# NikolasMarkou/blind_image_denoising

Hardware: AMD Instinct MI355X
Metric: denoised images/sec (256x256x3) + MAE vs ref, resnet_1x18 (higher is better)
Workload: dtype f16x2 split (hi+lo, fp32 accumulate)

## Files before the change

blind_image_denoising_amd/csrc/fused_h3w.hip:

```cpp
#include "h3v_core.h"
#include "h3_bands.h"
#include "base_rows.h"

#ifndef H3W_PRIO_SET
#define H3W_PRIO_SET 0
#endif
#if H3W_PRIO_SET == 1
#define H3W_PRIO_A1 0
#define H3W_PRIO_B1 1
#define H3W_PRIO_A2 2
#define H3W_PRIO_B2 3
#elif H3W_PRIO_SET == 2
#define H3W_PRIO_A1 3
#define H3W_PRIO_B1 2
#define H3W_PRIO_A2 1
#define H3W_PRIO_B2 0
#elif H3W_PRIO_SET == 3
#define H3W_PRIO_A1 0
#define H3W_PRIO_B1 2
#define H3W_PRIO_A2 0
#define H3W_PRIO_B2 2
#elif H3W_PRIO_SET == 4
#define H3W_PRIO_A1 2
#define H3W_PRIO_B1 0
#define H3W_PRIO_A2 2
#define H3W_PRIO_B2 0
#endif
#ifndef H3W_PRIO_A1
#define H3W_PRIO_A1 1
#endif
#ifndef H3W_PRIO_B1
#define H3W_PRIO_B1 1
#endif
#ifndef H3W_PRIO_A2
#define H3W_PRIO_A2 1
#endif
#ifndef H3W_PRIO_B2
#define H3W_PRIO_B2 1
#endif

#ifndef H3W_XCD_ORDER
#define H3W_XCD_ORDER 1
#endif

struct H3WGeom {
    static constexpr int NG = 9, GW = 16 * NG;
    static constexpr int G = 3;
    static constexpr int NR = 3, NW = 12, NT = 768;
    static constexpr int SW = 128;
    static constexpr int PITCH = (GW + 2) * 16;
    static constexpr int NRX0 = 5, NRM = 2, NRX1 = 3, NRO = 2;
    static constexpr int PD = 3;
    static constexpr int UNROLL = 6;
    static constexpr int X0_PLANE = (NRX0 * PITCH + 255) / 256 * 256, M_PLANE = (NRM * PITCH + 255) / 256 * 256;
    static constexpr int X1_PLANE = (NRX1 * PITCH + 255) / 256 * 256;
    static constexpr int OUT_PLANE = GW * 16, OUT_SLOT = 4 * OUT_PLANE;
    static constexpr int X0_OFF = 0, M1_OFF = X0_OFF + 4 * X0_PLANE, X1_OFF = M1_OFF + 4 * M_PLANE, M2_OFF = X1_OFF + 4 * X1_PLANE;
    static constexpr int OUT_OFF = M2_OFF + 4 * M_PLANE, LDS_BYTES = OUT_OFF + NRO * OUT_SLOT;
    static constexpr int BIN_RING = 4, BIN_ROWPX = GW + 4;
    static constexpr int BIN_SLOT = 2 * BIN_ROWPX * 8;
    static constexpr int BIN_OFF = LDS_BYTES, BWA_OFF = BIN_OFF + BIN_RING * BIN_SLOT, BINVS_OFF = BWA_OFF + 3 * 64 * 16;
    static constexpr int BRED_OFF = BINVS_OFF + 16, LDS_BYTES_BASE = BRED_OFF + NT * 4;
    static_assert(LDS_BYTES_BASE <= 160 * 1024 && BIN_OFF % 16 == 0 && BIN_SLOT % 16 == 0 && LDS_BYTES_BASE % 16 == 0, "LDS (producer)");
    static constexpr int LEAD = 12;
    static constexpr int NSTAMP = 4;
    static_assert(UNROLL % NRM == 0 && UNROLL % NRO == 0 && UNROLL % NRX1 == 0 && UNROLL % 3 == 0, "static slots");
    static_assert(NRX0 == PD + 2, "x0 ring: rows s-1 (residual), s (conv1a), s+1 (landed), s+2, s+3 (in flight)");
    static_assert(LDS_BYTES <= 160 * 1024, "LDS");
    static_assert(3 * X0_PLANE + NRX0 * PITCH < 65536, "fragment offsets fit the 16-bit ds offset");
};

struct H3WTile : BandUnit {
    int X0, X1;
    int G0;
    int D0, D1;
};

__device__ __forceinline__ H3WTile h3w_tile(const FusedH3WArgs& a, const int t)
{
    H3WTile r{bf_band_unit<H3W_XCD_ORDER != 0>(a, t)};
    r.X0 = r.sx * H3WGeom::SW;
    r.X1 = min(a.W, r.X0 + H3WGeom::SW);
    r.G0 = min(max(r.X0 - 8, 0), max(a.W - H3WGeom::GW, 0));
    r.D0 = max(0, (r.X0 - 4) & ~7);
    r.D1 = min(a.W, (r.X1 + 4 + 7) & ~7);
    return r;
}

template <int INP>
struct H3WRoleA {
    using Gm = H3WGeom;
    const char* tin;
    char* tmid;
    h8 w[13];
    f32x4 acc[Gm::G][3];
    int rp, rs;
    int wr;
    float inv_s, relu_floor;
    float lane_scale[Gm::G];
    bool skip_last = false;

    __device__ __forceinline__ void init(const void* wimg, const FusedH3WArgs& a, const float* aux, const int lane, const int gc0)
    {
        const int q = lane >> 4;
#pragma unroll
        for (int i = 0; i < 13; ++i) w[i] = reinterpret_cast<const h8*>(wimg)[bf_band_wimage(a, i) * 64 + lane];
        inv_s = aux[0];
        relu_floor = a.act1_relu ? 0.f : -__builtin_inff();
        rp = (q & 1) * INP + (gc0 + (q >> 1)) * 16;
        rs = ((q & 1) + 2 * (q >> 1)) * INP + (gc0 + 2) * 16;
        wr = (q >> 1) * Gm::M_PLANE + (gc0 + 1) * 16 + (q & 1) * 8;
#pragma unroll
        for (int g = 0; g < Gm::G; ++g)
#pragma unroll
            for (int k = 0; k < 3; ++k) acc[g][k] = (f32x4){0.f, 0.f, 0.f, 0.f};
    }
    __device__ __forceinline__ void set_tile(const H3WTile& t, const int W, const int gc0)
    {
#pragma unroll
        for (int g = 0; g < Gm::G; ++g) lane_scale[g] = (t.G0 + gc0 + 16 * g < W) ? inv_s : 0.f;
    }

    __device__ __forceinline__ H3VFrag load(const int islot_bytes, const int g) const
    {
        H3VFrag f;
        const char* p = tin + rp + islot_bytes;
        f.ph = *reinterpret_cast<const h8*>(p + g * 256);
        f.pl = *reinterpret_cast<const h8*>(p + g * 256 + 2 * INP);
        f.s = *reinterpret_cast<const h8*>(tin + rs + islot_bytes + g * 256);
        return f;
    }

    __device__ __forceinline__ H3VEpi<true> epilogue(const int g, const int mslot, const f32x4 v, const bool rowok) const
    {
        H3VEpi<true> e;
        e.v = v;
        e.sc = rowok ? lane_scale[g] : 0.f;
        e.floor_ = relu_floor;
        e.p = tmid + wr + mslot * Gm::PITCH + g * 256;
        e.lo_off = 2 * Gm::M_PLANE;
        return e;
    }

    template <int J, class Epi>
    __device__ __forceinline__ void mfmas(const int g, const int a1, const int a2, const H3VFrag& cur, f32x4& c0, Epi* epi)
    {
        if constexpr (J < 15) {
            constexpr int k = J / 3, which = J % 3;
            if (!(H3V_ABLATE & 8) && !(skip_last && g == Gm::G - 1)) {
                if constexpr (which == 0) acc[g][a2] = h3v_mfma(cur, w, 2, k, acc[g][a2]);
                else if constexpr (which == 1) acc[g][a1] = h3v_mfma(cur, w, 1, k, acc[g][a1]);
                else c0 = h3v_mfma(cur, w, 0, k, c0);
            } else if (J == 0) {
                acc[g][a2][0] += (float)cur.ph[0] + (float)cur.pl[1] + (float)cur.s[2];
            }
            __builtin_amdgcn_sched_barrier(0);
            if constexpr (J >= 2) {
                if (epi) epi->template pair<J - 2>();
            }
            mfmas<J + 1>(g, a1, a2, cur, c0, epi);
        }
    }

    template <int PH, class Hook>
    __device__ __forceinline__ void step(const int islot_bytes, const bool rowok, Hook& hook)
    {
        constexpr int a0 = PH % 3, a1 = (PH + 2) % 3, a2 = (PH + 1) % 3;
        constexpr int mslot = PH % Gm::NRM;
        H3VFrag cur = load(islot_bytes, 0);
#pragma unroll
        for (int g = 0; g < Gm::G; ++g) {
            H3VFrag nx;
            if (g + 1 < Gm::G) nx = load(islot_bytes, g + 1);
            __builtin_amdgcn_sched_barrier(0);
            f32x4 c0 = {0.f, 0.f, 0.f, 0.f};
            if (g > 0) {
                H3VEpi<true> e = epilogue(g - 1, mslot, acc[g - 1][a2], rowok);
                mfmas<0>(g, a1, a2, cur, c0, &e);
            } else {
                mfmas<0>(g, a1, a2, cur, c0, (H3VEpi<true>*)nullptr);
                hook.after_first_group();
                __builtin_amdgcn_sched_barrier(0);
            }
            acc[g][a0] = c0;
            if (g + 1 < Gm::G) cur = nx;
        }
        H3VEpi<true> e = epilogue(Gm::G - 1, mslot, bf_acc_ready(acc[Gm::G - 1][a2]), rowok);
        e.all();
    }
};

template <int RESP, int OUTP>
struct H3WRoleB {
    using Gm = H3WGeom;
    const char* tmid;
    const char* tres;
    char* tout;
    h8 w[13];
    f32x4 acc[Gm::G][3];
    int rp, rs;
    int rr;
    int wo;
    float inv_s2;
    f32x4 shs;
    float lane_scale[Gm::G];
    bool skip_last = false;

    __device__ __forceinline__ void init(const void* wimg, const FusedH3WArgs& a, const float* aux, const int lane, const int gc0,
                                         const bool out_is_ring)
    {
        const int q = lane >> 4;
#pragma unroll
        for (int i = 0; i < 13; ++i) w[i] = reinterpret_cast<const h8*>(wimg)[bf_band_wimage(a, i) * 64 + lane];
        inv_s2 = aux[48];
        shs = *reinterpret_cast<const f32x4*>(aux + 32 + q * 4) * (1.0f / inv_s2);
        rp = (q & 1) * Gm::M_PLANE + (gc0 + (q >> 1)) * 16;
        rs = ((q & 1) + 2 * (q >> 1)) * Gm::M_PLANE + (gc0 + 2) * 16;
        rr = ((q & 1) + 2 * (q >> 1)) * RESP + (gc0 + 1) * 16;
        wo = (q >> 1) * OUTP + (gc0 + (out_is_ring ? 1 : 0)) * 16 + (q & 1) * 8;
#pragma unroll
        for (int g = 0; g < Gm::G; ++g)
#pragma unroll
            for (int k = 0; k < 3; ++k) acc[g][k] = (f32x4){0.f, 0.f, 0.f, 0.f};
    }
    __device__ __forceinline__ void set_tile(const H3WTile& t, const int W, const int gc0)
    {
#pragma unroll
        for (int g = 0; g < Gm::G; ++g) lane_scale[g] = (t.G0 + gc0 + 16 * g < W) ? inv_s2 : 0.f;
    }

    __device__ __forceinline__ H3VFrag load(const int mslot, const int g) const
    {
        H3VFrag f;
        const int o = mslot * Gm::PITCH + g * 256;
        f.ph = *reinterpret_cast<const h8*>(tmid + rp + o);
        f.pl = *reinterpret_cast<const h8*>(tmid + rp + o + 2 * Gm::M_PLANE);
        f.s = *reinterpret_cast<const h8*>(tmid + rs + o);
        return f;
    }
    __device__ __forceinline__ h8 load_res(const int xslot_bytes, const int g) const
    {
        return *reinterpret_cast<const h8*>(tres + rr + xslot_bytes + g * 256);
    }

    __device__ __forceinline__ H3VEpi<false> epilogue(const int g, const int oslot_bytes, const f32x4 accv, const bool rowok) const
    {
        H3VEpi<false> e;
        e.v = accv;
        e.sc = rowok ? lane_scale[g] : 0.f;
        e.floor_ = 0.f;
        e.p = tout + wo + oslot_bytes + g * 256;
        e.lo_off = 2 * OUTP;
        return e;
    }

    template <int J, class Epi>
    __device__ __forceinline__ void mfmas(const int g, const int a1, const int a2, const H3VFrag& cur, const h8 xr, f32x4& c0, Epi* epi)
    {
        if constexpr (J < 16) {
            if (!(H3V_ABLATE & 4) && !(skip_last && g == Gm::G - 1)) {
                if constexpr (J == 0) {
                    c0 = MFMA_H(w[12], xr, shs);
                } else {
                    constexpr int k = (J - 1) / 3, which = (J - 1) % 3;
                    if constexpr (which == 0) acc[g][a2] = h3v_mfma(cur, w, 2, k, acc[g][a2]);
                    else if constexpr (which == 1) acc[g][a1] = h3v_mfma(cur, w, 1, k, acc[g][a1]);
                    else c0 = h3v_mfma(cur, w, 0, k, c0);
                }
            } else if (J == 0) {
                acc[g][a2][0] += (float)cur.ph[0] + (float)cur.pl[1] + (float)cur.s[2] + (float)xr[3];
            }
            __builtin_amdgcn_sched_barrier(0);
            if constexpr (J >= 2) {
                if (epi) epi->template pair<J - 2>();
            }
            mfmas<J + 1>(g, a1, a2, cur, xr, c0, epi);
        }
    }

    template <int PH, class Hook>
    __device__ __forceinline__ void step(const int xslot_bytes, const int oslot_bytes, const bool rowok, Hook& hook)
    {
        constexpr int mslot = (PH + 1) % Gm::NRM;
        constexpr int a0 = PH % 3, a1 = (PH + 2) % 3, a2 = (PH + 1) % 3;
        H3VFrag cur = load(mslot, 0);
        h8 xr = load_res(xslot_bytes, 0);
#pragma unroll
        for (int g = 0; g < Gm::G; ++g) {
            H3VFrag nx;
            h8 xn;
            if (g + 1 < Gm::G) {
                nx = load(mslot, g + 1);
                xn = load_res(xslot_bytes, g + 1);
            }
            __builtin_amdgcn_sched_barrier(0);
            f32x4 c0;
            if (g > 0) {
                H3VEpi<false> e = epilogue(g - 1, oslot_bytes, acc[g - 1][a2], rowok);
                mfmas<0>(g, a1, a2, cur, xr, c0, &e);
            } else {
                mfmas<0>(g, a1, a2, cur, xr, c0, (H3VEpi<false>*)nullptr);
                hook.after_first_group();
                __builtin_amdgcn_sched_barrier(0);
            }
            acc[g][a0] = c0;
            if (g + 1 < Gm::G) {
                cur = nx;
                xr = xn;
            }
        }
        H3VEpi<false> e = epilogue(Gm::G - 1, oslot_bytes, bf_acc_ready(acc[Gm::G - 1][a2]), rowok);
        e.all();
    }
};

#ifndef H3W_MEM_ROLES
#define H3W_MEM_ROLES 0
#endif
constexpr int h3w_mem_kind(const int role)
{
    constexpr int loader[4] = {2, 0, 1, 3}, storer[4] = {0, 1, 0, 0};
    return role == loader[H3W_MEM_ROLES] ? 1 : (role == storer[H3W_MEM_ROLES] ? 2 : 0);
}

template <int KIND>
struct H3WMem {
    __device__ __forceinline__ H3WMem(const FusedH3WArgs&, char*, const char*, int, unsigned) {}
    __device__ __forceinline__ void set_tile(const H3WTile&, int) {}
    __device__ __forceinline__ void prologue(const H3WTile&) {}
    __device__ __forceinline__ void begin(const H3WTile&, int, int) {}
    __device__ __forceinline__ void after_first_group() {}
    __device__ __forceinline__ void end() {}
    __device__ __forceinline__ void finish() {}
};

template <>
struct H3WMem<1> {
    using Gm = H3WGeom;
    const FusedH3WArgs& a;
    char* tin;
    int piece;
    unsigned plane_g;
    unsigned col_off;
    bool active;
    int dslot;

    __device__ __forceinline__ H3WMem(const FusedH3WArgs& a_, char* tx0, const char*, const int rw, const unsigned pg)
        : a(a_), tin(tx0), piece(rw), plane_g(pg), col_off(0), active(false), dslot(0) {}
    __device__ __forceinline__ void set_tile(const H3WTile& t, const int lane)
    {
        const int c = t.G0 + 64 * piece + lane;
        active = (c >= t.D0) & (c < t.D1) & (64 * piece + lane < Gm::GW);
        col_off = (unsigned)c * 16u;
    }
    __device__ __forceinline__ void dma_row(const H3WTile& t, const int r, const int slot) const
    {
        if (H3V_ABLATE & 1) return;
        const int y = t.y(r - 4);
        const bool ok = (y >= 0) & (y < a.H) & (r < t.nrows + 8);
#pragma unroll
        for (int plane = 0; plane < 4; ++plane) {
            const char* src = ok ? reinterpret_cast<const char*>(a.in) + t.img + (size_t)plane * plane_g + (size_t)y * a.W * 16 + col_off
                                 : reinterpret_cast<const char*>(a.zeros);
            char* dst = tin + plane * Gm::X0_PLANE + slot * Gm::PITCH + (1 + 64 * piece) * 16;
            if (active) h3_dma16(src, dst);
        }
    }
    static constexpr int INFLIGHT = 2 * 4;
    __device__ __forceinline__ void wait_landed() const { __builtin_amdgcn_s_waitcnt(h3_vmcnt((H3V_ABLATE & 1) ? 0 : INFLIGHT)); }
    __device__ __forceinline__ void prologue(const H3WTile& t)
    {
#pragma unroll
        for (int r = 0; r < Gm::PD; ++r) dma_row(t, r, r);
        wait_landed();
        dslot = Gm::PD;
    }
    __device__ __forceinline__ void begin(const H3WTile& t, const int s, int)
    {
        dma_row(t, s + Gm::PD, dslot);
        dslot = h3v_wrap(dslot + 1, Gm::NRX0);
    }
    __device__ __forceinline__ void after_first_group() {}
    __device__ __forceinline__ void end() { wait_landed(); }
    __device__ __forceinline__ void finish() { __builtin_amdgcn_s_waitcnt(h3_vmcnt(0)); }
};

template <>
struct H3WMem<2> {
    using Gm = H3WGeom;
    const FusedH3WArgs& a;
    const char* tout;
    int first, np;
    unsigned plane_g;
    int st_off[3];
    unsigned g_off[3];
    bool okc[3];
    h8 rec[3];
    bool have;
    char* image;
    size_t row_off;

    __device__ __forceinline__ H3WMem(const FusedH3WArgs& a_, char*, const char* tout_, const int rw, const unsigned pg)
        : a(a_), tout(tout_), first(3 * rw), np(rw < 2 ? 3 : 2), plane_g(pg), have(false), image(nullptr), row_off(0) {}
    __device__ __forceinline__ void set_tile(const H3WTile& t, const int lane)
    {
#pragma unroll
        for (int i = 0; i < 3; ++i) {
            const int p = first + i, plane = p >> 1, c = t.X0 + 64 * (p & 1) + lane;
            okc[i] = (i < np) & (c < t.X1);
            st_off[i] = plane * Gm::OUT_PLANE + (c - t.G0) * 16;
            g_off[i] = (unsigned)plane * plane_g + (unsigned)c * 16u;
        }
    }
    __device__ __forceinline__ void prologue(const H3WTile&) {}
    __device__ __forceinline__ void begin(const H3WTile& t, const int s, const int PH)
    {
        const int k = s - Gm::LEAD, oslot = (PH + 1) % Gm::NRO;
        have = (k >= 0) & (k < t.nrows) & !(H3V_ABLATE & 2);
        if (!have) return;
        image = reinterpret_cast<char*>(a.out) + t.img;
        row_off = (size_t)t.y(k) * a.W * 16;
#pragma unroll
        for (int i = 0; i < 3; ++i)
            if (i < np) rec[i] = *reinterpret_cast<const h8*>(tout + oslot * Gm::OUT_SLOT + st_off[i]);
    }
    __device__ __forceinline__ void after_first_group()
    {
        if (!have) return;
#pragma unroll
        for (int i = 0; i < 3; ++i)
            if (okc[i]) h3_stream_store16(image, 4u * plane_g, row_off, g_off[i], rec[i]);
    }
    __device__ __forceinline__ void end() {}
    __device__ __forceinline__ void finish() {}
};

template <>
struct H3WMem<3> {
    using Gm = H3WGeom;
    const FusedH3WArgs& a;
    const char* tout;
    int half;
    int st_off;
    int col;
    bool okc;

    __device__ __forceinline__ H3WMem(const FusedH3WArgs& a_, char*, const char* tout_, const int rw, const unsigned)
        : a(a_), tout(tout_), half(rw), st_off(0), col(0), okc(false) {}
    __device__ __forceinline__ void set_tile(const H3WTile& t, const int lane)
    {
        col = t.X0 + 64 * half + lane;
        okc = (half < 2) & (col < t.X1) & (col < a.Wo);
        st_off = (col - t.G0) * 16;
    }
    __device__ __forceinline__ void prologue(const H3WTile&) {}
    __device__ __forceinline__ void begin(const H3WTile& t, const int s, const int PH)
    {
        const int k = s - Gm::LEAD, oslot = (PH + 1) % Gm::NRO;
        bool have = (half < 2) & (k >= 0) & (k < t.nrows) & !(H3V_ABLATE & 2);
        if (have) have = t.y(k) < a.Ho;
        if (!have) return;
        char* orow = reinterpret_cast<char*>(a.head_out) + ((size_t)t.b * a.Ho + (size_t)t.y(k)) * a.Wo * 3 * (a.head_u8 ? 1 : 4);
        const char* src = tout + oslot * Gm::OUT_SLOT + st_off;
        float h0 = 0.f, h1 = 0.f, h2 = 0.f;
#pragma unroll
        for (int hf = 0; hf < 2; ++hf) {
            const h8 hi = *reinterpret_cast<const h8*>(src + hf * Gm::OUT_PLANE), lo = *reinterpret_cast<const h8*>(src + (2 + hf) * Gm::OUT_PLANE);
#pragma unroll
            for (int c = 0; c < 8; ++c) {
                const float v = (float)hi[c] + (float)lo[c];
                const f32x4 w = *reinterpret_cast<const f32x4*>(a.head_wh + (hf * 8 + c) * 4);
                h0 = fmaf(v, w.x, h0);
                h1 = fmaf(v, w.y, h1);
                h2 = fmaf(v, w.z, h2);
            }
        }
        const bool finite = fabsf(h0) <= 3.0e38f && fabsf(h1) <= 3.0e38f && fabsf(h2) <= 3.0e38f;
        if (!finite && a.status) atomicOr(a.status, BF_STATUS_F16_RANGE);
        float r[3] = {h0, h1, h2};
#pragma unroll
        for (int o = 0; o < 3; ++o) {
            float v = (1.0f - 2.0f / (__expf(4.0f * r[o]) + 1.0f)) * 0.51f;
            if (a.denormalize) v = (fminf(fmaxf(v, -0.5f), 0.5f) + 0.5f) * (a.v_max - a.v_min) + a.v_min;
            r[o] = v;
        }
        if (!okc) return;
        if (a.head_u8) {
            unsigned char* p = reinterpret_cast<unsigned char*>(orow) + (size_t)col * 3;
#pragma unroll
            for (int o = 0; o < 3; ++o) p[o] = (unsigned char)fminf(fmaxf(rintf(r[o]), 0.f), 255.f);
        } else {
            float* p = reinterpret_cast<float*>(orow) + (size_t)col * 3;
#pragma unroll
            for (int o = 0; o < 3; ++o) p[o] = r[o];
        }
        __builtin_amdgcn_sched_barrier(0);
    }
    __device__ __forceinline__ void after_first_group() {}
    __device__ __forceinline__ void end() {}
    __device__ __forceinline__ void finish() {}
};

#ifndef H3W_BASE_SPREAD
#define H3W_BASE_SPREAD 1
#endif
constexpr int h3w_base_groups(const int role)
{
    return H3W_BASE_SPREAD == 0 ? (role == 2 ? 3 : 0) : (H3W_BASE_SPREAD == 1 ? (role >= 1 ? 1 : 0) : (role <= 2 ? 1 : 0));
}
constexpr int h3w_base_first_group(const int role, const int rw)
{
    return H3W_BASE_SPREAD == 0 ? 3 * rw : (H3W_BASE_SPREAD == 1 ? 3 * (role - 1) + rw : 3 * role + rw);
}
constexpr bool h3w_base_fetches(const int role) { return role == 2; }

template <int NGW, bool FETCH>
struct H3WProducer {
    using Gm = H3WGeom;
    const FusedH3WArgs& a;
    char* tx0;
    char* tring;
    const char* twa;
    int g0, fw;
    float inv_s, floor_;
    int wr;
    int fo;
    int col0;
    int px, xcol;
    const uint8_t* img;
    unsigned raw[3];
    BrPixel rawp;
    int dslot;

    __device__ __forceinline__ H3WProducer(const FusedH3WArgs& a_, char* lds, const int g0_, const int fw_)
        : a(a_), tx0(lds + Gm::X0_OFF), tring(lds + Gm::BIN_OFF), twa(lds + Gm::BWA_OFF), g0(g0_), fw(fw_), wr(0), fo(0), col0(0),
          px(0), xcol(0), img(nullptr), raw{0u, 0u, 0u}, rawp{false, false}, dslot(0)
    {
        inv_s = *reinterpret_cast<const float*>(lds + Gm::BINVS_OFF);
        floor_ = a.base_relu ? 0.f : -__builtin_inff();
    }
    __device__ __forceinline__ void set_tile(const H3WTile& t, const int lane)
    {
        const int n = lane & 15, q = lane >> 4, gc0 = 16 * g0 + n;
        wr = (q >> 1) * Gm::X0_PLANE + (gc0 + 1) * 16 + (q & 1) * 8;
        const int p = gc0 + 2 * (q & 1);
        fo = ((p & 1) * Gm::BIN_ROWPX + (p & ~1)) * 8;
        twa = tx0 - Gm::X0_OFF + Gm::BWA_OFF + lane * 16;
        col0 = t.G0 + gc0;
        px = 64 * fw + lane;
        xcol = t.G0 - 1 + px;
        img = reinterpret_cast<const uint8_t*>(a.base_u8) + (size_t)t.b * a.Hs * a.Ws * 3;
    }
    __device__ __forceinline__ void request(const H3WTile& t, const int u)
    {
        const int yy = t.ybase + u - 5;
        const bool need = (px < Gm::GW + 2) & (u <= t.nrows + 9);
        rawp = br_pixel(yy, xcol, a.H, a.W, a.Hs, a.Ws);
        rawp.inside &= need;
        rawp.colour &= need;
        if (rawp.colour) {
            const uint8_t* p = img + ((size_t)yy * a.Ws + xcol) * 3;
            raw[0] = p[0];
            raw[1] = p[1];
            raw[2] = p[2];
        }
    }
    __device__ __forceinline__ void commit(const int u)
    {
        if (px >= Gm::GW + 2) return;
        const h4 v = br_record(rawp, raw[0], raw[1], raw[2]);
        h4* row = reinterpret_cast<h4*>(tring + (u & (Gm::BIN_RING - 1)) * Gm::BIN_SLOT);
        row[px] = v;
        if (px > 0) row[Gm::BIN_ROWPX + px - 1] = v;
    }
    __device__ __forceinline__ void produce(const H3WTile& t, const int r, const int slot)
    {
        if (r >= t.nrows + 8) return;
        const int y = t.y(r - 4);
        const bool rowok = (y >= 0) & (y < a.H);
        f32x4 acc[NGW];
#pragma unroll
        for (int g = 0; g < NGW; ++g) acc[g] = (f32x4){0.f, 0.f, 0.f, 0.f};
#pragma unroll
        for (int dy = 0; dy < 3; ++dy) {
            const h8 wa = *reinterpret_cast<const h8*>(twa + dy * 64 * 16);
            const char* row = tring + ((r + dy) & (Gm::BIN_RING - 1)) * Gm::BIN_SLOT + fo;
#pragma unroll
            for (int g = 0; g < NGW; ++g) acc[g] = MFMA_H(wa, *reinterpret_cast<const h8*>(row + g * 128), acc[g]);
        }
#pragma unroll
        for (int g = 0; g < NGW; ++g) {
            H3VEpi<true> e;
            e.v = bf_acc_ready(acc[g]);
            e.sc = (rowok & (col0 + 16 * g < a.W)) ? inv_s : 0.f;
            e.floor_ = floor_;
            e.p = tx0 + wr + slot * Gm::PITCH + g * 256;
            e.lo_off = 2 * Gm::X0_PLANE;
            e.all();
        }
    }
    __device__ __forceinline__ void fill(const H3WTile& t)
    {
        if constexpr (FETCH) {
#pragma unroll
            for (int u = 0; u < Gm::BIN_RING; ++u) {
                request(t, u);
                commit(u);
            }
            request(t, Gm::BIN_RING);
        }
    }
    __device__ __forceinline__ void prologue(const H3WTile& t)
    {
        produce(t, 0, 0);
        dslot = 1;
    }
    __device__ __forceinline__ void begin(const H3WTile& t, const int s)
    {
        if constexpr (FETCH) {
            commit(s + 4);
            request(t, s + 5);
        }
        produce(t, s + 1, dslot);
        dslot = h3v_wrap(dslot + 1, Gm::NRX0);
        __builtin_amdgcn_sched_barrier(0);
    }
};

template <>
struct H3WProducer<0, false> {
    __device__ __forceinline__ H3WProducer(const FusedH3WArgs&, char*, int, int) {}
    __device__ __forceinline__ void set_tile(const H3WTile&, int) {}
    __device__ __forceinline__ void fill(const H3WTile&) {}
    __device__ __forceinline__ void prologue(const H3WTile&) {}
    __device__ __forceinline__ void begin(const H3WTile&, int) {}
};

template <bool HEAD, bool BASE>
constexpr int h3w_hook_kind(const int role)
{
    const int k = h3w_mem_kind(role);
    return (HEAD && k == 2) ? 3 : ((BASE && k == 1) ? 0 : k);
}

template <bool HEAD, bool BASE>
__global__ __launch_bounds__(H3WGeom::NT, 3) void fused_block2_h3w_kernel(FusedH3WArgs a)
{
    using Gm = H3WGeom;
    extern __shared__ __attribute__((aligned(16))) char h3w_lds[];
    char* tx0 = h3w_lds + Gm::X0_OFF;
    char* tm1 = h3w_lds + Gm::M1_OFF;
    char* tx1 = h3w_lds + Gm::X1_OFF;
    char* tm2 = h3w_lds + Gm::M2_OFF;
    char* tout = h3w_lds + Gm::OUT_OFF;
    const int tid = threadIdx.x, lane = tid & 63;
    const int wave = __builtin_amdgcn_readfirstlane(tid >> 6);
    const int n = lane & 15;
    const int role = wave / Gm::NR, rw = wave - role * Gm::NR;
    const unsigned plane_g = (unsigned)a.H * (unsigned)a.W * 16u;
    const int gc0 = 16 * Gm::G * rw + n;

    if (BASE && a.status && blockIdx.x == 0 && tid == 0) *a.status = 0;
    for (int i = tid * 16; i < (BASE ? Gm::LDS_BYTES_BASE : Gm::LDS_BYTES); i += Gm::NT * 16)
        *reinterpret_cast<f32x4*>(h3w_lds + i) = (f32x4){0.f, 0.f, 0.f, 0.f};
    __syncthreads();
    if constexpr (BASE) {
        const float bs = br_weight_scale(a.base_w, reinterpret_cast<float*>(h3w_lds + Gm::BRED_OFF));
        if (wave == 0) {
#pragma unroll
            for (int dy = 0; dy < 3; ++dy)
                *reinterpret_cast<h8*>(h3w_lds + Gm::BWA_OFF + (dy * 64 + lane) * 16) = br_operand(a.base_w, bs, dy, lane);
            if (lane == 0) *reinterpret_cast<float*>(h3w_lds + Gm::BINVS_OFF) = 1.0f / bs;
        }
        __syncthreads();
    }

#if H3V_ABLATE & 32
    unsigned long long stamp_sum[Gm::NSTAMP] = {0, 0, 0, 0}, stamp_prev, real0;
    asm volatile("s_memrealtime %0\n\ts_memtime %1\n\ts_waitcnt lgkmcnt(0)" : "=s"(real0), "=s"(stamp_prev)::"memory");
#endif

#define H3W_ROW_IN_IMAGE(k) ((t.y(k) >= 0) & (t.y(k) < a.H))
#define H3W_BAND(R, M, P, ACTIVE, STEP)                                                                         \
    for (int ti = blockIdx.x; ti < a.ntiles; ti += gridDim.x) {                                               \
        const H3WTile t = h3w_tile(a, ti);                                                                    \
        R.set_tile(t, a.W, gc0);                                                                              \
        M.set_tile(t, lane);                                                                                  \
        P.set_tile(t, lane);                                                                                  \
        if constexpr (BASE) {                                      \
            P.fill(t);                                                                                        \
            h3v_barrier();                                                                                    \
        }                                                                                                     \
        P.prologue(t);                                                                                        \
        M.prologue(t);                                                                                        \
        h3v_barrier();                                                 \
        const int nsteps = t.nrows + Gm::LEAD;                                                                \
        int slot5 = 0;                                                                           \
        for (int s0 = 0; s0 < nsteps; s0 += Gm::UNROLL) {                                                     \
            H3W_ONE(0, M, P, ACTIVE, STEP); H3W_ONE(1, M, P, ACTIVE, STEP); H3W_ONE(2, M, P, ACTIVE, STEP);   \
            H3W_ONE(3, M, P, ACTIVE, STEP); H3W_ONE(4, M, P, ACTIVE, STEP); H3W_ONE(5, M, P, ACTIVE, STEP);   \
        }                                                                                                     \
        M.finish();                                                                                           \
        h3v_barrier();                                                                                        \
    }
#define H3W_ONE(PH, M, P, ACTIVE, STEP)                                                                         \
    do {                                                                                                      \
        const int s = s0 + PH;                                                                                \
        P.begin(t, s);                                                                                        \
        M.begin(t, s, PH);                                                                                    \
        if (ACTIVE(s)) { STEP(PH); }                                                                          \
        else M.after_first_group();                                                                           \
        slot5 = h3v_wrap(slot5 + 1, Gm::NRX0);                                                                \
        H3V_STAMP(0);                                                                                         \
        M.end();                                                                                              \
        H3V_STAMP(1);                                                                                         \
        h3v_barrier();                                                                                        \
        H3V_STAMP(2);                                                                                         \
    } while (0)

    if (role == 0) {
        __builtin_amdgcn_s_setprio(H3W_PRIO_A1);
        H3WRoleA<Gm::X0_PLANE> R;
        R.tin = tx0; R.tmid = tm1;
        R.init(a.w1r[0], a, a.aux[0], lane, gc0);
        R.skip_last = (H3V_ABLATE & 256) && rw == Gm::NR - 1;
        H3WMem<h3w_hook_kind<HEAD, BASE>(0)> M(a, tx0, tout, rw, plane_g);
        H3WProducer<BASE ? h3w_base_groups(0) : 0, BASE && h3w_base_groups(0) && h3w_base_fetches(0)> P(a, h3w_lds, h3w_base_first_group(0, rw), rw);
        __builtin_amdgcn_s_waitcnt(h3_vmcnt(0));
#define H3W_ACTIVE(s) ((s) < t.nrows + 8)
#define H3W_STEP(PH) R.template step<PH>(slot5 * Gm::PITCH, (s >= 2) & H3W_ROW_IN_IMAGE(s - 5), M)
        H3W_BAND(R, M, P, H3W_ACTIVE, H3W_STEP)
#undef H3W_ACTIVE
#undef H3W_STEP
    } else if (role == 1) {
        __builtin_amdgcn_s_setprio(H3W_PRIO_B1);
        H3WRoleB<Gm::X0_PLANE, Gm::X1_PLANE> R;
        R.tmid = tm1; R.tres = tx0; R.tout = tx1;
        R.init(a.w2r[0], a, a.aux[0], lane, gc0, true);
        R.skip_last = (H3V_ABLATE & 256) && rw == Gm::NR - 1;
        H3WMem<h3w_hook_kind<HEAD, BASE>(1)> M(a, tx0, tout, rw, plane_g);
        H3WProducer<BASE ? h3w_base_groups(1) : 0, BASE && h3w_base_groups(1) && h3w_base_fetches(1)> P(a, h3w_lds, h3w_base_first_group(1, rw), rw);
        __builtin_amdgcn_s_waitcnt(h3_vmcnt(0));
#define H3W_ACTIVE(s) (((s) >= 3) & ((s) < t.nrows + 9))
#define H3W_STEP(PH) R.template step<PH>(h3v_wrap(slot5 + Gm::NRX0 - 1, Gm::NRX0) * Gm::PITCH, (PH % Gm::NRX1) * Gm::PITCH, H3W_ROW_IN_IMAGE(s - 7), M)
        H3W_BAND(R, M, P, H3W_ACTIVE, H3W_STEP)
#undef H3W_ACTIVE
#undef H3W_STEP
    } else if (role == 2) {
        __builtin_amdgcn_s_setprio(H3W_PRIO_A2);
        H3WRoleA<Gm::X1_PLANE> R;
        R.tin = tx1; R.tmid = tm2;
        R.init(a.w1r[1], a, a.aux[1], lane, gc0);
        R.skip_last = (H3V_ABLATE & 256) && rw == Gm::NR - 1;
        H3WMem<h3w_hook_kind<HEAD, BASE>(2)> M(a, tx0, tout, rw, plane_g);
        H3WProducer<BASE ? h3w_base_groups(2) : 0, BASE && h3w_base_groups(2) && h3w_base_fetches(2)> P(a, h3w_lds, h3w_base_first_group(2, rw), rw);
        __builtin_amdgcn_s_waitcnt(h3_vmcnt(0));
#define H3W_ACTIVE(s) (((s) >= 6) & ((s) < t.nrows + 10))
#define H3W_STEP(PH) R.template step<PH>(((PH + 2) % Gm::NRX1) * Gm::PITCH, H3W_ROW_IN_IMAGE(s - 9), M)
        H3W_BAND(R, M, P, H3W_ACTIVE, H3W_STEP)
#undef H3W_ACTIVE
#undef H3W_STEP
    } else {
        __builtin_amdgcn_s_setprio(H3W_PRIO_B2);
        H3WRoleB<Gm::X1_PLANE, Gm::OUT_PLANE> R;
        R.tmid = tm2; R.tres = tx1; R.tout = tout;
        R.init(a.w2r[1], a, a.aux[1], lane, gc0, false);
        R.skip_last = (H3V_ABLATE & 256) && rw == Gm::NR - 1;
        H3WMem<h3w_hook_kind<HEAD, BASE>(3)> M(a, tx0, tout, rw, plane_g);
        H3WProducer<BASE ? h3w_base_groups(3) : 0, BASE && h3w_base_groups(3) && h3w_base_fetches(3)> P(a, h3w_lds, h3w_base_first_group(3, rw), rw);
        __builtin_amdgcn_s_waitcnt(h3_vmcnt(0));
#define H3W_ACTIVE(s) (((s) >= 9) & ((s) < t.nrows + 11))
#define H3W_STEP(PH) R.template step<PH>(((PH + 1) % Gm::NRX1) * Gm::PITCH, (PH % Gm::NRO) * Gm::OUT_SLOT, true, M)
        H3W_BAND(R, M, P, H3W_ACTIVE, H3W_STEP)
#undef H3W_ACTIVE
#undef H3W_STEP
    }
#undef H3W_BAND
#undef H3W_ONE
#undef H3W_ROW_IN_IMAGE
#if H3V_ABLATE & 32
    {
        unsigned long long real1;
        asm volatile("s_memrealtime %0\n\ts_waitcnt lgkmcnt(0)" : "=s"(real1)::"memory");
        stamp_sum[3] = real1 - real0;
    }
    if (a.dbg && lane == 0) {
        for (int k = 0; k < Gm::NSTAMP; ++k) a.dbg[((size_t)blockIdx.x * Gm::NW + wave) * 8 + k] = stamp_sum[k];
    }
#endif
}

bool bf_fused_block2_h3w_supports(int H, int W) { return W >= 1 && H >= 1; }

hipError_t bf_launch_fused_block2_h3w(const FusedH3WArgs& args, hipStream_t s)
{
    using Gm = H3WGeom;
    FusedH3WArgs a = args;
    if (!a.zeros || (!a.in && !a.base_u8) || (!a.out && !a.head_wh) || !bf_fused_block2_h3w_supports(a.H, a.W)) return hipErrorInvalidValue;
    if (a.base_u8 && (!a.base_w || a.head_wh || a.reverse_tiles || a.Hs < 1 || a.Ws < 1 || a.Hs > a.H || a.Ws > a.W)) return hipErrorInvalidValue;
    if ((int64_t)a.H * a.W * 64 >= ((int64_t)1 << 32)) return hipErrorInvalidValue;
    const BandPlan p = bf_band_plan(a.B, a.H, (a.W + Gm::SW - 1) / Gm::SW, Gm::LEAD + 2);
    a.nstrips = p.nstrips;
    a.rows_per_tile = p.rows_per_tile;
    a.tiles_y = p.tiles_y;
    a.ntiles = p.ntiles;
    if (a.head_wh && (!a.head_out || a.Ho < 1 || a.Wo < 1 || a.Ho > a.H || a.Wo > a.W)) return hipErrorInvalidValue;
    void (*kernel)(FusedH3WArgs) = a.base_u8 ? fused_block2_h3w_kernel<false, true>
                                   : a.head_wh ? fused_block2_h3w_kernel<true, false> : fused_block2_h3w_kernel<false, false>;
    const int lds = a.base_u8 ? Gm::LDS_BYTES_BASE : Gm::LDS_BYTES;
    const hipError_t e = bf_set_max_lds(reinterpret_cast<const void*>(kernel), lds);
    if (e != hipSuccess) return e;
    hipLaunchKernelGGL(kernel, dim3(p.grid), dim3(Gm::NT), lds, s, a);
    return hipGetLastError();
}
```

Baseline: 30560.

## Shadow base-layer producer MFMAs and epilogue into the first group's MFMA chain

The base-conv producer work, previously done as a standalone produce() per step, is now handed to the role's first-group MFMA sequence. It either runs as a precomputed epilogue interleaved with the MFMAs, or as staggered MFMAs with fragment reads slotted between them. This is meant to hide the producer's LDS reads, MFMAs and stores inside the otherwise epilogue-free first group. Optional late fetching of base pixels and a narrower raw-byte load are also added. The cost is more registers per wave (fragments, accumulator, epilogue state), which could reduce occupancy or add spills.

```diff
diff --git a/blind_image_denoising_amd/csrc/fused_h3w.hip b/blind_image_denoising_amd/csrc/fused_h3w.hip
--- a/blind_image_denoising_amd/csrc/fused_h3w.hip
+++ b/blind_image_denoising_amd/csrc/fused_h3w.hip
@@ -162,8 +162,8 @@
         }
     }
 
-    template <int PH, class Hook>
-    __device__ __forceinline__ void step(const int islot_bytes, const bool rowok, Hook& hook)
+    template <int PH, class Hook, class Prod>
+    __device__ __forceinline__ void step(const int islot_bytes, const bool rowok, Hook& hook, Prod& prod)
     {
         constexpr int a0 = PH % 3, a1 = (PH + 2) % 3, a2 = (PH + 1) % 3;
         constexpr int mslot = PH % Gm::NRM;
@@ -178,8 +178,9 @@
                 H3VEpi<true> e = epilogue(g - 1, mslot, acc[g - 1][a2], rowok);
                 mfmas<0>(g, a1, a2, cur, c0, &e);
             } else {
-                mfmas<0>(g, a1, a2, cur, c0, (H3VEpi<true>*)nullptr);
+                mfmas<0>(g, a1, a2, cur, c0, prod.shadow());
                 hook.after_first_group();
+                prod.after_first_group();
                 __builtin_amdgcn_sched_barrier(0);
             }
             acc[g][a0] = c0;
@@ -278,8 +279,8 @@
         }
     }
 
-    template <int PH, class Hook>
-    __device__ __forceinline__ void step(const int xslot_bytes, const int oslot_bytes, const bool rowok, Hook& hook)
+    template <int PH, class Hook, class Prod>
+    __device__ __forceinline__ void step(const int xslot_bytes, const int oslot_bytes, const bool rowok, Hook& hook, Prod& prod)
     {
         constexpr int mslot = (PH + 1) % Gm::NRM;
         constexpr int a0 = PH % 3, a1 = (PH + 2) % 3, a2 = (PH + 1) % 3;
@@ -299,8 +300,9 @@
                 H3VEpi<false> e = epilogue(g - 1, oslot_bytes, acc[g - 1][a2], rowok);
                 mfmas<0>(g, a1, a2, cur, xr, c0, &e);
             } else {
-                mfmas<0>(g, a1, a2, cur, xr, c0, (H3VEpi<false>*)nullptr);
+                mfmas<0>(g, a1, a2, cur, xr, c0, prod.shadow());
                 hook.after_first_group();
+                prod.after_first_group();
                 __builtin_amdgcn_sched_barrier(0);
             }
             acc[g][a0] = c0;
@@ -513,6 +515,13 @@
     return H3W_BASE_SPREAD == 0 ? 3 * rw : (H3W_BASE_SPREAD == 1 ? 3 * (role - 1) + rw : 3 * role + rw);
 }
 constexpr bool h3w_base_fetches(const int role) { return role == 2; }
+#ifndef H3W_BASE_SHADOW
+#define H3W_BASE_SHADOW 1
+#endif
+#ifndef H3W_BASE_FETCH_LATE
+#define H3W_BASE_FETCH_LATE 0
+#endif
+static_assert(H3W_BASE_SHADOW >= 0 && H3W_BASE_SHADOW <= 2 && (H3W_BASE_SHADOW == 0 || H3W_BASE_SPREAD != 0), "the shadowed producer: one group per wave");
 
 template <int NGW, bool FETCH>
 struct H3WProducer {
@@ -528,14 +537,24 @@
     int col0;
     int px, xcol;
     const uint8_t* img;
-    unsigned raw[3];
+    unsigned short raw01;
+    unsigned char raw2;
     BrPixel rawp;
     int dslot;
+    static constexpr bool LATE = FETCH && H3W_BASE_FETCH_LATE != 0;
+    static constexpr bool ASKS = H3W_BASE_SHADOW != 0 || LATE;
+    const H3WTile* tile;
+    int fs;
+    H3VEpi<true> e;
+    h8 wa[3], fb[3];
+    f32x4 pacc;
+    int in_row;
 
     __device__ __forceinline__ H3WProducer(const FusedH3WArgs& a_, char* lds, const int g0_, const int fw_)
         : a(a_), tx0(lds + Gm::X0_OFF), tring(lds + Gm::BIN_OFF), twa(lds + Gm::BWA_OFF), g0(g0_), fw(fw_), wr(0), fo(0), col0(0),
-          px(0), xcol(0), img(nullptr), raw{0u, 0u, 0u}, rawp{false, false}, dslot(0)
-    {
+          px(0), xcol(0), img(nullptr), raw01(0), raw2(0), rawp{false, false}, dslot(0), tile(nullptr), fs(0)
+    {
+        static_assert(H3W_BASE_SHADOW == 0 || NGW == 1, "the shadowed producer: one group per wave");
         inv_s = *reinterpret_cast<const float*>(lds + Gm::BINVS_OFF);
         floor_ = a.base_relu ? 0.f : -__builtin_inff();
     }
@@ -550,6 +569,7 @@
         px = 64 * fw + lane;
         xcol = t.G0 - 1 + px;
         img = reinterpret_cast<const uint8_t*>(a.base_u8) + (size_t)t.b * a.Hs * a.Ws * 3;
+        tile = &t;
     }
     __device__ __forceinline__ void request(const H3WTile& t, const int u)
     {
@@ -560,15 +580,14 @@
         rawp.colour &= need;
         if (rawp.colour) {
             const uint8_t* p = img + ((size_t)yy * a.Ws + xcol) * 3;
-            raw[0] = p[0];
-            raw[1] = p[1];
-            raw[2] = p[2];
+            __builtin_memcpy(&raw01, p, 2);
+            raw2 = p[2];
         }
     }
     __device__ __forceinline__ void commit(const int u)
     {
         if (px >= Gm::GW + 2) return;
-        const h4 v = br_record(rawp, raw[0], raw[1], raw[2]);
+        const h4 v = br_record(rawp, raw01 & 0xffu, raw01 >> 8, raw2);
         h4* row = reinterpret_cast<h4*>(tring + (u & (Gm::BIN_RING - 1)) * Gm::BIN_SLOT);
         row[px] = v;
         if (px > 0) row[Gm::BIN_ROWPX + px - 1] = v;
@@ -615,13 +634,71 @@
         produce(t, 0, 0);
         dslot = 1;
     }
-    __device__ __forceinline__ void begin(const H3WTile& t, const int s)
+    __device__ __forceinline__ void read_fragments(const int dy)
+    {
+        wa[dy] = *reinterpret_cast<const h8*>(twa + dy * 64 * 16);
+        fb[dy] = *reinterpret_cast<const h8*>(tring + ((in_row + dy) & (Gm::BIN_RING - 1)) * Gm::BIN_SLOT + fo);
+    }
+    __device__ __forceinline__ void hand_over(const H3WTile& t, const int r, const int slot)
+    {
+        const int y = t.y(r - 4);
+        const bool rowok = (y >= 0) & (y < a.H) & (r < t.nrows + 8);
+        e.sc = (rowok & (col0 < a.W)) ? inv_s : 0.f;
+        e.floor_ = floor_;
+        e.p = tx0 + wr + slot * Gm::PITCH;
+        e.lo_off = 2 * Gm::X0_PLANE;
+        in_row = r;
+#pragma unroll
+        for (int dy = 0; dy < (H3W_BASE_SHADOW == 2 ? 1 : 3); ++dy) read_fragments(dy);
+        if constexpr (H3W_BASE_SHADOW == 1) {
+            f32x4 acc = {0.f, 0.f, 0.f, 0.f};
+#pragma unroll
+            for (int dy = 0; dy < 3; ++dy) acc = MFMA_H(wa[dy], fb[dy], acc);
+            e.v = acc;
+        }
+    }
+    template <int SLOT> __device__ __forceinline__ void pair()
+    {
+        if constexpr (H3W_BASE_SHADOW == 1) {
+            e.template pair<SLOT>();
+        } else if constexpr (SLOT == 0 || SLOT == 2 || SLOT == 4) {
+            const f32x4 zero = {0.f, 0.f, 0.f, 0.f};
+            pacc = MFMA_H(wa[SLOT / 2], fb[SLOT / 2], SLOT == 0 ? zero : pacc);
+            __builtin_amdgcn_sched_barrier(0);
+            if constexpr (SLOT < 4) {
+                read_fragments(SLOT / 2 + 1);
+                __builtin_amdgcn_sched_barrier(0);
+            }
+        } else if constexpr (SLOT == 6) {
+            e.v = pacc;
+            e.template pair<0>();
+        } else if constexpr (SLOT > 6) {
+            e.template pair<SLOT - 6>();
+        }
+    }
+    __device__ __forceinline__ auto shadow()
+    {
+        if constexpr (H3W_BASE_SHADOW != 0) return this;
+        else return (H3VEpi<true>*)nullptr;
+    }
+    __device__ __forceinline__ void after_first_group()
+    {
+        if constexpr (LATE) {
+            commit(fs + 4);
+            request(*tile, fs + 5);
+        }
+    }
+    __device__ __forceinline__ void begin(const H3WTile& t, const int s, const bool active)
     {
         if constexpr (FETCH) {
-            commit(s + 4);
-            request(t, s + 5);
-        }
-        produce(t, s + 1, dslot);
+            if (!LATE || !active) {
+                commit(s + 4);
+                request(t, s + 5);
+            }
+            fs = s;
+        }
+        if (H3W_BASE_SHADOW != 0 && active) hand_over(t, s + 1, dslot);
+        else produce(t, s + 1, dslot);
         dslot = h3v_wrap(dslot + 1, Gm::NRX0);
         __builtin_amdgcn_sched_barrier(0);
     }
@@ -633,7 +710,10 @@
     __device__ __forceinline__ void set_tile(const H3WTile&, int) {}
     __device__ __forceinline__ void fill(const H3WTile&) {}
     __device__ __forceinline__ void prologue(const H3WTile&) {}
-    __device__ __forceinline__ void begin(const H3WTile&, int) {}
+    static constexpr bool ASKS = false;
+    __device__ __forceinline__ void begin(const H3WTile&, int, bool) {}
+    __device__ __forceinline__ H3VEpi<true>* shadow() { return nullptr; }
+    __device__ __forceinline__ void after_first_group() {}
 };
 
 template <bool HEAD, bool BASE>
@@ -706,7 +786,7 @@
 #define H3W_ONE(PH, M, P, ACTIVE, STEP)                                                                         \
     do {                                                                                                      \
         const int s = s0 + PH;                                                                                \
-        P.begin(t, s);                                                                                        \
+        P.begin(t, s, decltype(P)::ASKS && (ACTIVE(s)));                                                      \
         M.begin(t, s, PH);                                                                                    \
         if (ACTIVE(s)) { STEP(PH); }                                                                          \
         else M.after_first_group();                                                                           \
@@ -728,7 +808,7 @@
         H3WProducer<BASE ? h3w_base_groups(0) : 0, BASE && h3w_base_groups(0) && h3w_base_fetches(0)> P(a, h3w_lds, h3w_base_first_group(0, rw), rw);
         __builtin_amdgcn_s_waitcnt(h3_vmcnt(0));
 #define H3W_ACTIVE(s) ((s) < t.nrows + 8)
-#define H3W_STEP(PH) R.template step<PH>(slot5 * Gm::PITCH, (s >= 2) & H3W_ROW_IN_IMAGE(s - 5), M)
+#define H3W_STEP(PH) R.template step<PH>(slot5 * Gm::PITCH, (s >= 2) & H3W_ROW_IN_IMAGE(s - 5), M, P)
         H3W_BAND(R, M, P, H3W_ACTIVE, H3W_STEP)
 #undef H3W_ACTIVE
 #undef H3W_STEP
@@ -742,7 +822,7 @@
         H3WProducer<BASE ? h3w_base_groups(1) : 0, BASE && h3w_base_groups(1) && h3w_base_fetches(1)> P(a, h3w_lds, h3w_base_first_group(1, rw), rw);
         __builtin_amdgcn_s_waitcnt(h3_vmcnt(0));
 #define H3W_ACTIVE(s) (((s) >= 3) & ((s) < t.nrows + 9))
-#define H3W_STEP(PH) R.template step<PH>(h3v_wrap(slot5 + Gm::NRX0 - 1, Gm::NRX0) * Gm::PITCH, (PH % Gm::NRX1) * Gm::PITCH, H3W_ROW_IN_IMAGE(s - 7), M)
+#define H3W_STEP(PH) R.template step<PH>(h3v_wrap(slot5 + Gm::NRX0 - 1, Gm::NRX0) * Gm::PITCH, (PH % Gm::NRX1) * Gm::PITCH, H3W_ROW_IN_IMAGE(s - 7), M, P)
         H3W_BAND(R, M, P, H3W_ACTIVE, H3W_STEP)
 #undef H3W_ACTIVE
 #undef H3W_STEP
@@ -756,7 +836,7 @@
         H3WProducer<BASE ? h3w_base_groups(2) : 0, BASE && h3w_base_groups(2) && h3w_base_fetches(2)> P(a, h3w_lds, h3w_base_first_group(2, rw), rw);
         __builtin_amdgcn_s_waitcnt(h3_vmcnt(0));
 #define H3W_ACTIVE(s) (((s) >= 6) & ((s) < t.nrows + 10))
-#define H3W_STEP(PH) R.template step<PH>(((PH + 2) % Gm::NRX1) * Gm::PITCH, H3W_ROW_IN_IMAGE(s - 9), M)
+#define H3W_STEP(PH) R.template step<PH>(((PH + 2) % Gm::NRX1) * Gm::PITCH, H3W_ROW_IN_IMAGE(s - 9), M, P)
         H3W_BAND(R, M, P, H3W_ACTIVE, H3W_STEP)
 #undef H3W_ACTIVE
 #undef H3W_STEP
@@ -770,7 +850,7 @@
         H3WProducer<BASE ? h3w_base_groups(3) : 0, BASE && h3w_base_groups(3) && h3w_base_fetches(3)> P(a, h3w_lds, h3w_base_first_group(3, rw), rw);
         __builtin_amdgcn_s_waitcnt(h3_vmcnt(0));
 #define H3W_ACTIVE(s) (((s) >= 9) & ((s) < t.nrows + 11))
-#define H3W_STEP(PH) R.template step<PH>(((PH + 1) % Gm::NRX1) * Gm::PITCH, (PH % Gm::NRO) * Gm::OUT_SLOT, true, M)
+#define H3W_STEP(PH) R.template step<PH>(((PH + 1) % Gm::NRX1) * Gm::PITCH, (PH % Gm::NRO) * Gm::OUT_SLOT, true, M, P)
         H3W_BAND(R, M, P, H3W_ACTIVE, H3W_STEP)
 #undef H3W_ACTIVE
 #undef H3W_STEP
```

After: 30690 (median of 6 runs). No clear change (+0.4%).
